# PABannier/biogpt.cpp

Measured on AMD Instinct MI355X. Metric: decode tokens/sec BioGPT Q4_0 n_ctx=1024, higher is better.
Workload: dtype int8; 1 GPU; greedy 200-token continuation of a 4-token prompt per GPU (main.cpp loop, -b 8, --top_k 1), BioGPT-base Q4_0, F32 KV cache, n_ctx=1024; 1 step = 1 continuation per rank; n_layer=24, d_model=1024, d_ff=4096, n_vocab=42384, n_predict=200, n_prompt=4, parallelism=replicas x1 (weights RCCL-broadcast once)

## Files before the change

### biogpt.cpp_amd/csrc/kernels_xpipe.hip.h

```cpp
#pragma once

#include "kernels_decode.hip.h"

namespace bgk {

typedef unsigned long long xp_u64;
typedef float xp_v4f __attribute__((ext_vector_type(4)));
#define XP_RLX __ATOMIC_RELAXED, __HIP_MEMORY_SCOPE_AGENT
constexpr uint32_t XP_SPIN_MAX = 400000u;

struct XpLayer {
    const float *ln0_w, *ln0_b, *ln1_w, *ln1_b;
    const float *bqkv, *bo, *b1, *b2;
    DevMatrix Wqkv, Wo, W1, W2;
    float *kcache, *vcache;
    unsigned long long *gx1, *gx;
};

constexpr int XP_G_QKV = 0;
constexpr int XP_G_ATT = 3072;
constexpr int XP_G_X1 = XP_G_ATT + 320;
constexpr int XP_G_H = XP_G_X1 + 1024;
constexpr int XP_G_X = XP_G_H + 1280;
constexpr int XP_G_LAYER = XP_G_X + 1024;
// ... 288 lines not shown
constexpr int XP_S_G = XP_S_PART + 256 * DEC_PS * 4;
constexpr int XP_S_LN = XP_S_G + 512;
constexpr int XP_S_BIAS = XP_S_LN + 16384;
constexpr int XP_S_CUR = XP_S_BIAS + 1536;
constexpr int XP_S_S = XP_S_CUR + 768;
constexpr int XP_S_REDF = XP_S_S + 1024;
constexpr int XP_S_REDD = XP_S_REDF + 512;
constexpr int XP_S_PV = XP_S_REDD + 128;
constexpr int XP_S_TOTAL = XP_S_PV + 8192;
static_assert(32 * DEC_PS2 <= 256 * DEC_PS, "fc2 block terms fit the shared region");
__host__ __device__ inline size_t xpipe_smem_bytes(int gelu_entries) { return XP_S_TOTAL + (size_t)gelu_entries * 2; }

template <int WT, bool EXPAND>
__device__ __forceinline__ float xp_dot(const Unit<WT> &u, const uint32_t *xq, float xd, float xs_f, int xs_i) {
    if constexpr (EXPAND) return unit_dot_settled<WT>(u, xq, xd, xs_f, xs_i);
    else return unit_dot_quant<WT>(u, xq, xd, xs_f, xs_i);
}
template <int WT, bool EXPAND>
__device__ __forceinline__ void xp_settle(Unit<WT> &u) {
    if constexpr (EXPAND) {
        settle_unit<WT>(u);
        asm volatile("" : "+v"(u.q0.x), "+v"(u.q0.y), "+v"(u.q0.z), "+v"(u.q0.w), "+v"(u.q1.x), "+v"(u.q1.y), "+v"(u.q1.z), "+v"(u.q1.w), "+v"(u.sc));
    }
}

__device__ __forceinline__ uint32_t xp_wave_sum_u32(uint32_t v) {
    int s = (int)v;
    s += dpp_i<DPP_QUAD_XOR1>(s); s += dpp_i<DPP_QUAD_XOR2>(s); s += dpp_i<DPP_ROW_HALF_MIRROR>(s); s += dpp_i<DPP_ROW_MIRROR>(s);
    return (uint32_t)((__builtin_amdgcn_readlane(s, 0) + __builtin_amdgcn_readlane(s, 16)) + (__builtin_amdgcn_readlane(s, 32) + __builtin_amdgcn_readlane(s, 48)));
}

template <int WT, int LPK, int NW, int KCAP, int ROLE, bool SPLIT, bool RES>
__device__ __forceinline__ void xp_run(const XpParams &p, unsigned char *smem, const int xcd, const int slot, const uint32_t epoch0, const int n_past0,
                                       const int n_gen0) {
    using TI = TypeInfo<WT>;
    static_assert(TI::quant && (WT != W_Q8_0 || SPLIT), "18-30 weight units per lane must fit the register file (Q8_0: 9 registers per unit: split layers)");
    static_assert(ROLE == 0 || ROLE == 1 || (ROLE == 2 && SPLIT), "0 attention head, 1 q/k/v rows, 2 (split layers) the MLP half");
    static_assert(SPLIT || TI::q81, "the producers publish Q8_0 block sums only for Q4_1 / Q5_1 (want_sum = q81): the symmetric formats need the signed units of the split form (unit_dot_settled)");
    constexpr bool ATTN = ROLE == 0;
    constexpr bool EXPAND = SPLIT;
    constexpr bool FIRST = !SPLIT || ROLE != 2, SECOND = !SPLIT || ROLE == 2;
    static_assert(LPK == 2 || LPK == 4 || LPK == 8 || LPK == 16, "lanes per key");
    static_assert(NW == 8 || NW == 16, "waves per workgroup");
    constexpr int D = 1024, DK = 64, NT = NW * 64;
    constexpr int QS = 96 / NW, OS = 16 / NW, FS = 64 / NW, F2R = 32 / NW;
    constexpr bool DUAL = SPLIT && KCAP > 256;
    constexpr int KW = DUAL ? KCAP / 2 : KCAP;
    constexpr int HI = (DUAL && ROLE == 1) ? 1 : 0;
    static_assert(KW % NW == 0 && KW <= NW * 64 / LPK, "key capacity of the launch");
    constexpr int NF4 = 16 / LPK, NV = KW / NW;
    float *const s_x = reinterpret_cast<float *>(smem + XP_S_X);
    float *const s_x1 = reinterpret_cast<float *>(smem + XP_S_X1);
    uint32_t *const s_xq = reinterpret_cast<uint32_t *>(smem + XP_S_XQ);
    float *const s_xd = reinterpret_cast<float *>(smem + XP_S_XD);
    uint32_t *const s_xs = reinterpret_cast<uint32_t *>(smem + XP_S_XS);
    double *const s_red = reinterpret_cast<double *>(smem + XP_S_RED);
    uint32_t *const s_hq = reinterpret_cast<uint32_t *>(smem + XP_S_HQ);
    float *const s_hd = reinterpret_cast<float *>(smem + XP_S_HD);
    uint32_t *const s_hs = reinterpret_cast<uint32_t *>(smem + XP_S_HS);
    float *const s_part = reinterpret_cast<float *>(smem + XP_S_PART);
    float *const s_g = reinterpret_cast<float *>(smem + XP_S_G);
    float *const s_ln = reinterpret_cast<float *>(smem + XP_S_LN);
    float *const s_bias = reinterpret_cast<float *>(smem + XP_S_BIAS);
    float *const s_cur = reinterpret_cast<float *>(smem + XP_S_CUR);
    float *const s_S = reinterpret_cast<float *>(smem + XP_S_S);
    float *const s_redf = reinterpret_cast<float *>(smem + XP_S_REDF);
    int *const s_redi = reinterpret_cast<int *>(smem + XP_S_REDF + 256);
    double *const s_redd = reinterpret_cast<double *>(smem + XP_S_REDD);
    double *const s_pv = reinterpret_cast<double *>(smem + XP_S_PV);
    uint16_t *const s_gelu = reinterpret_cast<uint16_t *>(smem + XP_S_TOTAL);
    uint32_t *const s_dead = reinterpret_cast<uint32_t *>(smem + XP_S_REDD + 96);
    uint32_t *const s_kvdead = reinterpret_cast<uint32_t *>(smem + XP_S_REDD + 64);
    uint32_t *const s_spec = reinterpret_cast<uint32_t *>(smem + XP_S_REDD + 112);
    const int t_cap = p.t_cap;
    const int n_units = SPLIT ? 2 * p.n_layer : p.n_layer;
    const int last_xcd = (n_units - 1) & 7;
    for (int tk = 0; tk < p.n_tok; tk++) {
    const uint32_t epoch = epoch0 + (uint32_t)tk;
    uint32_t etag = epoch;
    const int n_past = n_past0 + tk, T = n_past + 1;
    if (tk > 0 && __hip_atomic_load(p.ctl + 1, XP_RLX) != 0u) break;
    for (int U = xcd; U < n_units; U += 8) {
        const int L = SPLIT ? (U >> 1) : U;
        int tid = threadIdx.x;
        asm volatile("" : "+v"(tid));
        const int lane = tid & 63, wave = tid >> 6;
        const int sub = lane & 31, rsub = lane >> 5;
        const bool worker = tid < 256;
        if (tk == 0 && U == xcd && U >= 2) {
            if (tid == 0) {
                const xp_u64 *g = SPLIT ? (ROLE != 2 ? XPL(L - 1).gx1 : XPL(L - 1).gx) : XPL(L - 2).gx;
                for (uint32_t spins = 0;; spins++) {
                    if ((uint32_t)(__hip_atomic_load(g, XP_RLX) >> 32) == epoch) break;
                    if (spins >= XP_SPIN_MAX) { xp_fail(p, 3u); break; }
                    if ((spins & 255u) == 255u && __hip_atomic_load(p.ctl + 1, XP_RLX) != 0u) break;
                    __builtin_amdgcn_s_sleep(16);
                }
            }
            __syncthreads();
        }
        const XpLayerK &Y = XPL(L);
        xp_u64 *const G = p.gran + (size_t)L * XP_G_LAYER;
        constexpr bool attn_wg = ATTN || (DUAL && ROLE == 1);
        const int head = slot & 15;
        Unit<WT> wo[OS], w1[FS], w2[F2R][2];
        {
            float4 l0 = make_float4(0.f, 0.f, 0.f, 0.f), l1 = l0, l2 = l0, l3 = l0;
            if (worker) {
                if (FIRST) { l0 = xp_ldg4(Y.ln0_w, tid); l1 = xp_ldg4(Y.ln0_b, tid); }
                if (SECOND) { l2 = xp_ldg4(Y.ln1_w, tid); l3 = xp_ldg4(Y.ln1_b, tid); }
            }
            float bv = 0.0f;
            if (tid < 192) { if (FIRST) bv = ((xp_gf)Y.bqkv)[(tid >> 6) * 1024 + head * 64 + (tid & 63)]; }
            else if (tid < 224) { if (FIRST) bv = ((xp_gf)Y.bo)[slot * 32 + tid - 192]; }
            else if (tid < 352) { if (SECOND) bv = ((xp_gf)Y.b1)[slot * 128 + tid - 224]; }
            else if (tid < 384) { if (SECOND) bv = ((xp_gf)Y.b2)[slot * 32 + tid - 352]; }
            if (FIRST) {
#pragma unroll
                for (int s = 0; s < OS; s++) load_unit<WT>(wo[s], XPL_MATRIX(Y.Wo), (int64_t)(slot * 32 + s * 2 * NW + wave * 2 + rsub) * 32 + sub);
            }
            if (SECOND) {
#pragma unroll
                for (int s = 0; s < FS; s++) load_unit<WT>(w1[s], XPL_MATRIX(Y.W1), (int64_t)(slot * 128 + s * 2 * NW + wave * 2 + rsub) * 32 + sub);
#pragma unroll
                for (int r = 0; r < F2R; r++)
#pragma unroll
                    for (int it = 0; it < 2; it++) load_unit<WT>(w2[r][it], XPL_MATRIX(Y.W2), (int64_t)(slot * 32 + wave * F2R + r) * 128 + lane + 64 * it);
            }
            if (worker) {
                if (FIRST) { reinterpret_cast<float4 *>(s_ln)[tid] = l0; reinterpret_cast<float4 *>(s_ln + 1024)[tid] = l1; }
                if (SECOND) { reinterpret_cast<float4 *>(s_ln + 2048)[tid] = l2; reinterpret_cast<float4 *>(s_ln + 3072)[tid] = l3; }
            }
            if (tid < 384) s_bias[tid] = bv;
            if constexpr (EXPAND) {
                if (FIRST) {
#pragma unroll
                    for (int s = 0; s < OS; s++) xp_settle<WT, EXPAND>(wo[s]);
                }
                if (SECOND) {
#pragma unroll
                    for (int s = 0; s < FS; s++) xp_settle<WT, EXPAND>(w1[s]);
#pragma unroll
                    for (int r = 0; r < F2R; r++) { xp_settle<WT, EXPAND>(w2[r][0]); xp_settle<WT, EXPAND>(w2[r][1]); }
                }
            }
        }
        auto layer_input = [&]() -> float4 {
            float4 xv = make_float4(0.f, 0.f, 0.f, 0.f);
            if (L == 0) {
                int tok;
                const bool emb_fast = XPK(tok_emb.type) == WT && XPK(pos_emb.type) == WT;
                uint32_t pq = 0u, psc = 0u, pqh = 0u;
                if (emb_fast && worker) xp_row4_request<WT>(XPK_MATRIX(pos_emb), n_past + 2, tid, pq, psc, pqh);
                auto sample_prev = [&]() __attribute__((always_inline)) -> int {
                    float bv = -INFINITY;
                    int bi = 0x7fffffff;
                    {
                        uint32_t v[4] = {0u, 0u, 0u, 0u};
                        const bool a0 = tid < XPK(lm_blocks), a1 = tid + NT < XPK(lm_blocks);
                        const uint32_t prev = epoch - 1u;
                        for (uint32_t spins = 0; !RES || etag != 0u; spins++) {
                            bool ok = true;
                            if (a0) {
                                const xp_u64 x0 = __hip_atomic_load(XPK(samp) + tid, XP_RLX), x1 = __hip_atomic_load(XPK(samp) + 1024 + tid, XP_RLX);
                                v[0] = (uint32_t)x0; v[1] = (uint32_t)x1;
                                ok &= (uint32_t)(x0 >> 32) == prev && (uint32_t)(x1 >> 32) == prev;
                            }
                            if (a1) {
                                const xp_u64 x0 = __hip_atomic_load(XPK(samp) + tid + NT, XP_RLX), x1 = __hip_atomic_load(XPK(samp) + 1024 + tid + NT, XP_RLX);
                                v[2] = (uint32_t)x0; v[3] = (uint32_t)x1;
                                ok &= (uint32_t)(x0 >> 32) == prev && (uint32_t)(x1 >> 32) == prev;
                            }
                            if (__all(ok)) break;
                            if (spins >= XP_SPIN_MAX) { if (lane == 0) xp_fail(p, 4u); if (RES) etag = 0u; break; }
                            if ((spins & (RES ? 255u : 1023u)) == (RES ? 255u : 1023u) && __any(__hip_atomic_load(p.ctl + 1, XP_RLX) != 0u)) { if (RES) etag = 0u; break; }
                            
                        }
                        if (a0) { bv = __uint_as_float(v[0]); bi = (int)v[1]; }
                        if (a1) {
                            const float ov = __uint_as_float(v[2]);
                            const int oi = (int)v[3];
                            if (ov > bv || (ov == bv && oi < bi)) { bv = ov; bi = oi; }
                        }
                    }
                    xp_argmax_wave(bv, bi);
                    if (lane == 0) { s_redf[wave] = bv; s_redi[wave] = bi; }
                    __syncthreads();
                    bv = s_redf[0]; bi = s_redi[0];
#pragma unroll
                    for (int w = 1; w < NW; w++)
                        if (s_redf[w] > bv || (s_redf[w] == bv && s_redi[w] < bi)) { bv = s_redf[w]; bi = s_redi[w]; }
                    if (bi < 0 || bi >= XPK(n_vocab)) bi = 0;
                    return bi;
                };
                if (RES && p.resident != 0 && tk == 0 && slot == 0 && tid == 0) { s_spec[0] = (uint32_t)XPK(res_spec0); s_spec[1] = 0xffffffffu; }
                if (RES && p.resident != 0 && tk > 0) {
                    xp_u64 *const gt = XPK(samp) + 2048;
                    if (slot == 0) {
                        unsigned long long *const wl4 = ((XPK(res_dbg) & 32) && XPK(wall) && tid == 0) ? XPK(wall) + 32768 + (size_t)((XPK(mbox_seq0) + (uint32_t)tk) & 4095u) * 4 : nullptr;
                        if (wl4) wl4[0] = wall_clock64();
                        const uint32_t want = XPK(mbox_seq0) + (uint32_t)tk;
                        auto wait_post = [&](uint32_t seq, int np, int &spec) __attribute__((always_inline)) -> int {
                            const xp_u64 *mb = reinterpret_cast<const xp_u64 *>(XPK(mbox)) + (size_t)(seq & 63u) * 4;
                            const unsigned long long t0 = wall_clock64();
                            for (;;) {
                                const xp_u64 w = __hip_atomic_load(mb, __ATOMIC_RELAXED, __HIP_MEMORY_SCOPE_SYSTEM);
                                if ((uint32_t)(w >> 40) == (seq & 0xffffffu)) {
                                    const int tv = (int)(w & 0xffffffu), pn = (int)((w >> 24) & 0x1fffu);
                                    spec = (int)((w >> 37) & 1u);
                                    return (pn == np && tv < XPK(n_vocab)) ? tv : -1;
                                }
                                if (wall_clock64() - t0 > (unsigned long long)XPK(idle_ticks)) return -1;
                                if (__hip_atomic_load(p.ctl + 1, XP_RLX) != 0u) return -1;
                                if (!(XPK(res_dbg) & 2)) __builtin_amdgcn_s_sleep(4);
                            }
                        };
                        if (tid == 0) {
                            const int pending = (int)s_spec[1];
                            int unused = 0;
                            s_spec[2] = (etag != 0u && (pending < 0 || wait_post(want - 1u, n_past - 1, unused) == pending)) ? 1u : 0u;
                        }
                        const int guess = sample_prev();
                        __syncthreads();
                        if (wl4) wl4[1] = wall_clock64();
                        if (tid == 0 && etag != 0u) {
                            int spec = (int)s_spec[0];
                            const bool ahead = (int)s_spec[1] >= 0 || spec != 0;
                            int got = -1;
                            if (s_spec[2] != 0u) {
                                if (XPK(spec_rec)) __hip_atomic_store(XPK(spec_rec), ((unsigned long long)want << 32) | (unsigned long long)(uint32_t)guess, __ATOMIC_RELAXED, __HIP_MEMORY_SCOPE_SYSTEM);
                                got = ahead ? guess : wait_post(want, n_past, spec);
                            }
                            if (got >= 0) {
                                xp_put_local(gt, epoch, (uint32_t)got);
                                xp_put(gt + 1, epoch, 1u);
                                s_spec[0] = (uint32_t)spec; s_spec[1] = ahead ? (uint32_t)guess : 0xffffffffu;
                            } else xp_quit(p);
                            if ((XPK(res_dbg) & 32) && XPK(wall)) XPK(wall)[(size_t)(want & 4095u) * 2] = wall_clock64();
                            if (wl4) wl4[2] = wall_clock64();
                        }
                    }
                    uint32_t v[1];
                    xp_sweep_q<RES, 1>(gt, true, epoch, v, p, etag);
                    tok = (int)v[0];
                    if (tok < 0 || tok >= XPK(n_vocab)) tok = 0;
                } else if (tk > 0) {
                    tok = sample_prev();
                    if (slot == 0 && tid == 0) {
                        int32_t *tokens = state_tokens(XPK(st));
                        const int g = n_gen0 + tk;
                        if (g < XPK(n_positions)) tokens[XPK(n_positions) + g] = tok;
                        tokens[0] = tok;
                    }
                    __syncthreads();
                } else if (XPK(tok_src) == 2) {
                    float bv = -INFINITY;
                    int bi = 0x7fffffff;
                    for (int k = tid; k < XPK(nparts); k += NT) {
                        const float v = XPK(pmax_val)[k];
                        const int ix = XPK(pmax_idx)[k];
                        if (v > bv || (v == bv && ix < bi)) { bv = v; bi = ix; }
                    }
    #pragma unroll
                    for (int off = 32; off > 0; off >>= 1) {
                        const float ov = __shfl_xor(bv, off, 64);
                        const int oi = __shfl_xor(bi, off, 64);
                        if (ov > bv || (ov == bv && oi < bi)) { bv = ov; bi = oi; }
                    }
                    if (lane == 0) { s_redf[wave] = bv; s_redi[wave] = bi; }
                    __syncthreads();
                    bv = s_redf[0]; bi = s_redi[0];
    #pragma unroll
                    for (int w = 1; w < NW; w++)
                        if (s_redf[w] > bv || (s_redf[w] == bv && s_redi[w] < bi)) { bv = s_redf[w]; bi = s_redi[w]; }
                    tok = bi;
                    if (tok < 0 || tok >= XPK(n_vocab)) tok = 0;
                    if (slot == 0 && tid == 0) {
                        int32_t *tokens = state_tokens(XPK(st));
                        const int g = n_gen0;
                        if (g < XPK(n_positions)) tokens[XPK(n_positions) + g] = tok;
                        tokens[0] = tok;
                    }
                } else {
                    tok = (RES && p.resident != 0) ? XPK(res_tok0) : state_tokens(XPK(st))[0];
                }
                if (slot == 0) XP_TAIL(tk, 5);
                if (worker) {
                    float e[4];
                    if (emb_fast) {
                        uint32_t tq, tsc, tqh;
                        xp_row4_request<WT>(XPK_MATRIX(tok_emb), tok, tid, tq, tsc, tqh);
                        float te[4], pe[4];
                        xp_row4_values<WT>(pq, psc, pqh, tid, pe);
                        xp_row4_values<WT>(tq, tsc, tqh, tid, te);
    #pragma unroll
                        for (int j = 0; j < 4; j++) e[j] = __fadd_rn(__fmul_rn(te[j], XPK(embed_scale)), pe[j]);
                    } else {
    #pragma unroll
                        for (int j = 0; j < 4; j++)
                            e[j] = __fadd_rn(__fmul_rn(dequant_elem(XPK_MATRIX(tok_emb), tok, 4 * tid + j), XPK(embed_scale)), dequant_elem(XPK_MATRIX(pos_emb), n_past + 2, 4 * tid + j));
                    }
                    xv = make_float4(e[0], e[1], e[2], e[3]);
                }
            } else if (wave < 4) {
                uint32_t v[4];
                xp_sweep_q<RES, 4, 256, true>(XPL(L - 1).gx + tid, true, epoch, v, p, etag);
                xv = make_float4(__uint_as_float(v[0]), __uint_as_float(v[1]), __uint_as_float(v[2]), __uint_as_float(v[3]));
            }
            if (RES && wave < 4 && lane == 0) { s_dead[wave] = (etag == 0u) ? 1u : 0u; }
            return xv;
        };
        if constexpr (FIRST) {
        constexpr bool MERGE = SPLIT && KCAP <= 128;
        if (!attn_wg && MERGE) {
            const float4 xv = layer_input();
            if (worker) reinterpret_cast<float4 *>(s_x)[tid] = xv;
            XP_WALL(0);
        }
        if (!attn_wg && !MERGE) {
            constexpr int Q0 = (KCAP <= 192) ? QS / 3 : 0;
            Unit<WT> wqkv[QS];
#pragma unroll
            for (int s = Q0; s < QS; s++) {
                const int jj = s * 2 * NW + wave * 2 + rsub;
                load_unit<WT>(wqkv[s], XPL_MATRIX(Y.Wqkv), (int64_t)((jj >> 6) * 1024 + head * 64 + (jj & 63)) * 32 + sub);
            }
#pragma unroll
            for (int s = Q0; s < QS; s++) xp_settle<WT, EXPAND>(wqkv[s]);
            const float4 xv = layer_input();
            XP_WALL(0);
            float4 lnw = xv, lnb = xv;
            if (worker) {
                reinterpret_cast<float4 *>(s_x)[tid] = xv;
                lnw = reinterpret_cast<const float4 *>(s_ln)[tid]; lnb = reinterpret_cast<const float4 *>(s_ln + 1024)[tid];
            }
            ln4_q8_1024<TI::q81, TI::q81>(xv, lnw, lnb, p.eps, s_red, s_xq, s_xd, s_xs);
            XP_WALL(6);
            uint32_t ax[8];
            const uint4 a = *reinterpret_cast<const uint4 *>(s_xq + sub * 8), b = *reinterpret_cast<const uint4 *>(s_xq + sub * 8 + 4);
            ax[0] = a.x; ax[1] = a.y; ax[2] = a.z; ax[3] = a.w; ax[4] = b.x; ax[5] = b.y; ax[6] = b.z; ax[7] = b.w;
            const float axd = s_xd[sub];
            const uint32_t axs = s_xs[sub];
            float *const part = s_part + wave * 2 * QS * DEC_PS;
#pragma unroll
            for (int s = Q0; s < QS; s++) part[(s * 2 + rsub) * DEC_PS + sub] = xp_dot<WT, EXPAND>(wqkv[s], ax, axd, __uint_as_float(axs), (int)axs);
            __builtin_amdgcn_fence(__ATOMIC_RELEASE, "wavefront");
            __builtin_amdgcn_wave_barrier();
            __builtin_amdgcn_fence(__ATOMIC_ACQUIRE, "wavefront");
            if (lane >= 2 * Q0 && lane < 2 * QS) {
                const int jj = (lane >> 1) * 2 * NW + wave * 2 + (lane & 1);
                float v = __fadd_rn(s_bias[jj], sum32_in_order(part + lane * DEC_PS));
                const int which = jj >> 6, d = jj & 63;
                if (which == 0) v = __fmul_rn(v, p.q_scale);
                xp_put_local(G + XP_G_QKV + which * 1024 + head * 64 + d, etag, __float_as_uint(v));
                if (which != 0 && (!RES || (etag != 0u && (s_dead[0] | s_dead[1] | s_dead[2] | s_dead[3]) == 0u))) {
                    float *kc_ = Y.kcache, *vc_ = Y.vcache;
                    asm volatile("" : "+s"(kc_), "+s"(vc_));
                    ((__attribute__((address_space(1))) float *)((which == 1) ? kc_ : vc_))[((size_t)head * p.P + n_past) * DK + d] = v;
                }
            }
            XP_WALL(1);
        }
        if (attn_wg) {
            float4 kr[NF4];
            float vr[NV];
            const int ksub = tid & (LPK - 1), kidx = tid / LPK;
            const int dd = tid & (DK - 1), sl = tid >> 6;
            {
                constexpr bool KV_SC1 = !MERGE;
                const float *kb = Y.kcache + (size_t)head * p.P * DK, *vb = Y.vcache + (size_t)head * p.P * DK;
                const __amdgpu_buffer_rsrc_t krs = xp_kv_rsrc(kb, p.P * DK * 4), vrs = xp_kv_rsrc(vb, p.P * DK * 4);
                if (KV_SC1 || kidx < t_cap) {
#pragma unroll
                    for (int m = 0; m < NF4; m++) kr[m] = xp_kv_load4<KV_SC1>(krs, kb, ((HI * KW + kidx) * (DK / 4) + ksub + LPK * m) * 4);
                } else {
#pragma unroll
                    for (int m = 0; m < NF4; m++) kr[m] = make_float4(0.f, 0.f, 0.f, 0.f);
                }
#pragma unroll
                for (int k = 0; k < NV; k++) {
                    const int j = HI * KW + sl + NW * k;
                    vr[k] = (KV_SC1 || j < t_cap) ? xp_kv_load1<KV_SC1>(vrs, vb, j * DK + dd) : 0.0f;
                }
            }
            if constexpr (MERGE) {
                Unit<WT> wqkv[QS];
#pragma unroll
                for (int s = 0; s < QS; s++) {
                    const int jj = s * 2 * NW + wave * 2 + rsub;
                    load_unit<WT>(wqkv[s], XPL_MATRIX(Y.Wqkv), (int64_t)((jj >> 6) * 1024 + head * 64 + (jj & 63)) * 32 + sub);
                }
#pragma unroll
                for (int s = 0; s < QS; s++) xp_settle<WT, EXPAND>(wqkv[s]);
                const float4 xv = layer_input();
                XP_WALL(0);
                if (L == 0 && slot == 0) { asm volatile("" :: "v"(xv.x)); XP_TAIL(tk, 6); }
                float4 lnw = xv, lnb = xv;
                if (worker) {
// ... 338 lines not shown
            if (lane < 2 * OS) {
                const int lr = (lane >> 1) * 2 * NW + wave * 2 + (lane & 1), row = slot * 32 + lr;
                const float v = __fadd_rn(__fadd_rn(sum32_in_order(part + lane * DEC_PS), s_bias[192 + lr]), s_x[row]);
                if (SPLIT) xp_put(Y.gx1 + xp_col_slot(row), etag, __float_as_uint(v));
                else xp_put_local(Y.gx1 + xp_col_slot(row), etag, __float_as_uint(v));
            }
        }
        XP_WALL(3);
        }
        if constexpr (SECOND) {
        float4 x1v = make_float4(0.f, 0.f, 0.f, 0.f), lnw = x1v, lnb = x1v;
        if (wave < 4) {
            uint32_t v[4];
            xp_sweep_q<RES, 4, 256, true>(Y.gx1 + tid, true, epoch, v, p, etag);
            x1v = make_float4(__uint_as_float(v[0]), __uint_as_float(v[1]), __uint_as_float(v[2]), __uint_as_float(v[3]));
            reinterpret_cast<float4 *>(s_x1)[tid] = x1v;
            XP_WALL(9);
            lnw = reinterpret_cast<const float4 *>(s_ln + 2048)[tid]; lnb = reinterpret_cast<const float4 *>(s_ln + 3072)[tid];
        }
        ln4_q8_1024<TI::q81, TI::q81>(x1v, lnw, lnb, p.eps, s_red, s_xq, s_xd, s_xs);
        XP_WALL(10);
        {
            uint32_t ax[8];
            const uint4 a = *reinterpret_cast<const uint4 *>(s_xq + sub * 8), b = *reinterpret_cast<const uint4 *>(s_xq + sub * 8 + 4);
            ax[0] = a.x; ax[1] = a.y; ax[2] = a.z; ax[3] = a.w; ax[4] = b.x; ax[5] = b.y; ax[6] = b.z; ax[7] = b.w;
            const float axd = s_xd[sub];
            const uint32_t axs = s_xs[sub];
            float *const part = s_part + wave * 2 * FS * DEC_PS;
#pragma unroll
            for (int s = 0; s < FS; s++) part[(s * 2 + rsub) * DEC_PS + sub] = xp_dot<WT, EXPAND>(w1[s], ax, axd, __uint_as_float(axs), (int)axs);
            __builtin_amdgcn_fence(__ATOMIC_RELEASE, "wavefront");
            __builtin_amdgcn_wave_barrier();
            __builtin_amdgcn_fence(__ATOMIC_ACQUIRE, "wavefront");
            if (lane < 2 * FS) {
                const int jr = (lane >> 1) * 2 * NW + wave * 2 + (lane & 1);
                const float v = __fadd_rn(s_bias[224 + jr], sum32_in_order(part + lane * DEC_PS));
                const uint32_t ix = f2h(v), neg = ix - 0x8000u;
                uint16_t g16;
                if (ix < (uint32_t)p.gelu_p) g16 = s_gelu[ix];
                else if (ix <= 0x7C00u) g16 = (p.gelu_p > 0) ? (uint16_t)ix : p.gelu_tab[ix];
                else if (neg < (uint32_t)p.gelu_n) g16 = s_gelu[p.gelu_p + neg];
                else if (neg < 0x7C00u && p.gelu_n > 0) g16 = (uint16_t)p.gelu_z;
                else g16 = p.gelu_tab[ix];
                s_g[jr] = h2f(g16);
            }
        }
        __syncthreads();
        XP_WALL(11);
        if (tid < 128) {
            int8_t q8; float d8; uint32_t s8;
            q8_block32(s_g[tid], TI::q81, q8, d8, s8, TI::q81);
            const uint32_t packed = xp_pack4(q8);
            const int blk = slot * 4 + (tid >> 5);
            if ((tid & 3) == 0) xp_put_local(G + XP_G_H + slot * 32 + (tid >> 2), etag, packed);
            if ((tid & 31) == 0) { xp_put_local(G + XP_G_H + 1024 + blk, etag, __float_as_uint(d8)); if (TI::q81) xp_put_local(G + XP_G_H + 1152 + blk, etag, s8); }
        }
        XP_WALL(4);
        {
            constexpr int NQ = 1024 / NT;
            uint32_t v[NQ + 1];
#pragma unroll
            for (int k = 0; k <= NQ; k++) v[k] = 0u;
            const xp_u64 *g = G + XP_G_H + tid;
            const bool tail = tid < (TI::q81 ? 256 : 128);
            for (uint32_t spins = 0; !RES || etag != 0u; spins++) {
                bool ok = true;
#pragma unroll
                for (int k = 0; k < NQ; k++) {
                    const xp_u64 a = __hip_atomic_load(g + k * NT, XP_RLX);
                    v[k] = (uint32_t)a;
                    ok &= (uint32_t)(a >> 32) == epoch;
                }
                if (tail) {
                    const xp_u64 a = __hip_atomic_load(g + 1024, XP_RLX);
                    v[NQ] = (uint32_t)a;
                    ok &= (uint32_t)(a >> 32) == epoch;
                }
                if (__all(ok)) break;
                if (spins >= XP_SPIN_MAX) { if (lane == 0) xp_fail(p, 1u); if (RES) etag = 0u; break; }
                if ((spins & (RES ? 255u : 1023u)) == (RES ? 255u : 1023u) && __any(__hip_atomic_load(p.ctl + 1, XP_RLX) != 0u)) { if (RES) etag = 0u; break; }
                
            }
#pragma unroll
            for (int k = 0; k < NQ; k++) s_hq[tid + k * NT] = v[k];
            if (tid < 128) s_hd[tid] = __uint_as_float(v[NQ]);
            else if (tid < 256) s_hs[tid - 128] = v[NQ];
        }
        __syncthreads();
        XP_WALL(12);
        {
            float *const part = s_part + wave * F2R * DEC_PS2;
#pragma unroll
            for (int it = 0; it < 2; it++) {
                const int u = lane + 64 * it;
                uint32_t ax[8];
                const uint4 a = *reinterpret_cast<const uint4 *>(s_hq + u * 8), b = *reinterpret_cast<const uint4 *>(s_hq + u * 8 + 4);
                ax[0] = a.x; ax[1] = a.y; ax[2] = a.z; ax[3] = a.w; ax[4] = b.x; ax[5] = b.y; ax[6] = b.z; ax[7] = b.w;
                const float axd = s_hd[u];
                const uint32_t axs = s_hs[u];
#pragma unroll
                for (int r = 0; r < F2R; r++) part[r * DEC_PS2 + u] = xp_dot<WT, EXPAND>(w2[r][it], ax, axd, __uint_as_float(axs), (int)axs);
            }
            __builtin_amdgcn_fence(__ATOMIC_RELEASE, "wavefront");
            __builtin_amdgcn_wave_barrier();
            __builtin_amdgcn_fence(__ATOMIC_ACQUIRE, "wavefront");
            if (lane < F2R) {
                const float4 *p4 = reinterpret_cast<const float4 *>(part + lane * DEC_PS2);
                float sumf = 0.0f;
#pragma unroll
                for (int b0 = 0; b0 < 32; b0 += 8) {
                    float4 t[8];
#pragma unroll
                    for (int j = 0; j < 8; j++) t[j] = p4[b0 + j];
#pragma unroll
                    for (int j = 0; j < 8; j++) {
                        sumf = __fadd_rn(sumf, t[j].x); sumf = __fadd_rn(sumf, t[j].y);
                        sumf = __fadd_rn(sumf, t[j].z); sumf = __fadd_rn(sumf, t[j].w);
                    }
                }
                const int lr = wave * F2R + lane, row = slot * 32 + lr;
                const float v = __fadd_rn(__fadd_rn(sumf, s_bias[352 + lr]), s_x1[row]);
                xp_put(Y.gx + xp_col_slot(row), etag, __float_as_uint(v));
                if (L == p.n_layer - 1) XPK(x_final)[row] = v;
            }
        }
        XP_WALL(5);
        if (L == p.n_layer - 1 && slot == 0) XP_TAIL(tk, 0);
        }
        __syncthreads();
    }
    const int lm_rank = xp_lm_rank(xcd, slot, n_units);
    if (p.lm != 0 && lm_rank >= 0 && lm_rank * 4 < XPK(lm_blocks)) {
        int tid = threadIdx.x;
        asm volatile("" : "+v"(tid));
        const int lane = tid & 63, wave = tid >> 6;
        const int sub = lane & 31, rsub = lane >> 5;
        const bool worker = tid < 256;
        constexpr int LMS = 128 / NW;
        const int row0 = lm_rank * 256;
        const bool alt = RES && p.resident != 0 && ((XPK(mbox_seq0) + (uint32_t)tk) & 1u) != 0u;
        float *const lg_dev = alt ? XPK(logits_alt) : XPK(logits);
        float *const lg_host = alt ? XPK(logits_host_alt) : XPK(logits_host);
        Unit<WT> wl[LMS];
#pragma unroll
        for (int s = 0; s < LMS; s++) {
            const int row = row0 + s * 2 * NW + wave * 2 + rsub;
            if (row < XPK(n_vocab)) load_unit<WT>(wl[s], XPK_MATRIX(Wlm), (int64_t)row * 32 + sub);
            else { wl[s].q0 = make_uint4(0u, 0u, 0u, 0u); wl[s].q1 = wl[s].q0; wl[s].sc = 0u; wl[s].qh = 0u; }
        }
#pragma unroll
        for (int s = 0; s < LMS; s++) xp_settle<WT, EXPAND>(wl[s]);
        float4 xv = make_float4(0.f, 0.f, 0.f, 0.f), lnw = xv, lnb = xv;
        if (worker) { lnw = reinterpret_cast<const float4 *>(XPK(lm_ln_w))[tid]; lnb = reinterpret_cast<const float4 *>(XPK(lm_ln_b))[tid]; }
        if (RES && p.resident != 0 && tk > 0 && !(XPK(res_dbg) & 64)) {
            uint32_t go[1];
            xp_sweep_q<RES, 1>(XPK(samp) + 2049, lane == 0, epoch, go, p, etag);
        }
        if (wave < 4) {
            uint32_t v[4];
            xp_sweep_q<RES, 4, 256, true>(XPL(p.n_layer - 1).gx + tid, true, epoch, v, p, etag);
            xv = make_float4(__uint_as_float(v[0]), __uint_as_float(v[1]), __uint_as_float(v[2]), __uint_as_float(v[3]));
            if (lm_rank == 0) XP_TAIL(tk, 1);
        }
        ln4_q8_1024<TI::q81, TI::q81>(xv, lnw, lnb, p.eps, s_red, s_xq, s_xd, s_xs);
        if (lm_rank == 0) XP_TAIL(tk, 2);
        uint32_t ax[8];
        const uint4 a = *reinterpret_cast<const uint4 *>(s_xq + sub * 8), b = *reinterpret_cast<const uint4 *>(s_xq + sub * 8 + 4);
        ax[0] = a.x; ax[1] = a.y; ax[2] = a.z; ax[3] = a.w; ax[4] = b.x; ax[5] = b.y; ax[6] = b.z; ax[7] = b.w;
        const float axd = s_xd[sub];
        const uint32_t axs = s_xs[sub];
        float *const part = s_part + wave * 2 * LMS * DEC_PS;
#pragma unroll
        for (int s = 0; s < LMS; s++) part[(s * 2 + rsub) * DEC_PS + sub] = xp_dot<WT, EXPAND>(wl[s], ax, axd, __uint_as_float(axs), (int)axs);
        __builtin_amdgcn_fence(__ATOMIC_RELEASE, "wavefront");
        __builtin_amdgcn_wave_barrier();
        __builtin_amdgcn_fence(__ATOMIC_ACQUIRE, "wavefront");
        float best_val = -INFINITY;
        int best_idx = 0x7fffffff;
        if (lane < 2 * LMS) {
            const int row = row0 + (lane >> 1) * 2 * NW + wave * 2 + (lane & 1);
            if (row < XPK(n_vocab)) {
                const float v = sum32_in_order(part + lane * DEC_PS);
                if constexpr (RES) s_S[row - row0] = v;
                else { XPK(logits)[row] = v; if (XPK(logits_host)) XPK(logits_host)[row] = v; }
                best_val = v; best_idx = row;
            }
        }
        if (lm_rank == 0) XP_TAIL(tk, 3);
        static_assert(64 / NW == 8 || 64 / NW == 4, "finisher lanes per block");
        xp_argmax_dpp<DPP_QUAD_XOR1>(best_val, best_idx); xp_argmax_dpp<DPP_QUAD_XOR2>(best_val, best_idx);
        if (64 / NW == 8) xp_argmax_dpp<DPP_ROW_HALF_MIRROR>(best_val, best_idx);
        constexpr int LPB = 64 / NW;
        if (lane < 2 * LMS && (lane & (LPB - 1)) == 0) { s_redf[(lane / LPB) * NW + wave] = best_val; s_redi[(lane / LPB) * NW + wave] = best_idx; }
        bool row_ok = true;
        if constexpr (RES) row_ok = __syncthreads_and(etag != 0u);
        else __syncthreads();
        if (RES && lg_host && wave == 1 && row_ok) {
            const int r = row0 + 4 * lane;
            if (XPK(res_dbg) & 4) {
            } else if (r + 3 < XPK(n_vocab)) {
                const xp_v4f v4 = *reinterpret_cast<const xp_v4f *>(s_S + 4 * lane);
                asm volatile("global_store_dwordx4 %0, %1, off sc0 sc1" :: "v"(lg_host + r), "v"(v4) : "memory");
                *reinterpret_cast<xp_v4f *>(lg_dev + r) = v4;
            } else {
                for (int j = r; j < XPK(n_vocab); j++) { __hip_atomic_store(lg_host + j, s_S[j - row0], __ATOMIC_RELAXED, __HIP_MEMORY_SCOPE_SYSTEM); lg_dev[j] = s_S[j - row0]; }
            }
            if (p.resident != 0) {
                if (lane < 4 && lm_rank * 4 + lane < XPK(lm_blocks)) {
                    float bm = s_redf[lane * NW];
#pragma unroll
                    for (int w = 1; w < NW; w++) bm = fmaxf(bm, s_redf[lane * NW + w]);
                    __hip_atomic_store(lg_host + xp_blockmax_offset(XPK(n_vocab)) + lm_rank * 4 + lane, bm, __ATOMIC_RELAXED, __HIP_MEMORY_SCOPE_SYSTEM);
                }
                if (!(XPK(res_dbg) & 1)) asm volatile("s_waitcnt vmcnt(0)" ::: "memory");
                if (lane == 0) __hip_atomic_store(XPK(done_host) + lm_rank, XPK(mbox_seq0) + (uint32_t)tk, __ATOMIC_RELAXED, __HIP_MEMORY_SCOPE_SYSTEM);
                if ((XPK(res_dbg) & 32) && XPK(wall) && lane == 0 && lm_rank == 0) XPK(wall)[(size_t)((XPK(mbox_seq0) + (uint32_t)tk) & 4095u) * 2 + 1] = wall_clock64();
                if ((XPK(res_dbg) & 32) && XPK(wall) && lane == 0) XPK(wall)[8192 + (size_t)((XPK(mbox_seq0) + (uint32_t)tk) & 63u) * 256 + lm_rank] = wall_clock64();
            }
        }
        if (tid < 4) {
            float bv = s_redf[tid * NW];
            int bi = s_redi[tid * NW];
#pragma unroll
            for (int w = 1; w < NW; w++) {
                const float ov = s_redf[tid * NW + w];
                const int oi = s_redi[tid * NW + w];
                if (ov > bv || (ov == bv && oi < bi)) { bv = ov; bi = oi; }
            }
            const int blk = lm_rank * 4 + tid;
            if (blk < XPK(lm_blocks)) {
                if (RES && !row_ok) {}
                else if (RES && alt) { XPK(pmax_alt_val)[blk] = bv; XPK(pmax_alt_idx)[blk] = bi; }
                else { XPK(pmax_out_val)[blk] = bv; XPK(pmax_out_idx)[blk] = bi; }
                if (tk + 1 < p.n_tok) {
                    xp_put(XPK(samp) + blk, etag, __float_as_uint(bv));
                    xp_put(XPK(samp) + 1024 + blk, etag, (uint32_t)bi);
                }
                if (RES && (XPK(res_dbg) & 32) && XPK(wall) && blk == 0) XPK(wall)[32768 + (size_t)((XPK(mbox_seq0) + (uint32_t)tk) & 4095u) * 4 + 3] = wall_clock64();
            }
        }
        if (lm_rank == 0) XP_TAIL(tk, 4);
        __syncthreads();
    }
    }
    if (threadIdx.x == 0) {
        if (xcd == last_xcd && slot == 0) {
            if (epoch0 + (uint32_t)p.n_tok > 0xF0000000u) xp_fail(p, 5u);
            __hip_atomic_store(p.ctl, epoch0 + (uint32_t)p.n_tok, XP_RLX);
            __hip_atomic_store(p.ctl + 2, __hip_atomic_load(p.ctl + 2, XP_RLX) + 1u, XP_RLX);
        }
        if (xcd == (last_xcd == 1 ? 2 : 1) && slot == 0 && p.adv != 0) { XPK(st)->n_past = n_past0 + p.n_tok; XPK(st)->n_gen = n_gen0 + p.n_tok; }
    }
}

template <int WT, int LPK, int NW, int KCAP, bool SPLIT, bool RES = false>
__global__ __launch_bounds__(NW * 64) void dec_xpipe_kernel(const XpParams p) {
    using TI = TypeInfo<WT>;
    static_assert(TI::quant && (WT != W_Q8_0 || SPLIT), "Q8_0 (9 registers per weight unit) runs with split layers");
    static_assert(LPK == 2 || LPK == 4 || LPK == 8 || LPK == 16, "lanes per key");
    static_assert(NW == 8 || NW == 16, "waves per workgroup");
    constexpr int D = 1024, DK = 64, NT = NW * 64;
    constexpr int QS = 96 / NW, OS = 16 / NW, FS = 64 / NW, F2R = 32 / NW;
    static_assert(KCAP % NW == 0 && (KCAP > 256 ? KCAP / 2 : KCAP) <= NW * 64 / LPK, "key capacity of the launch");
    constexpr int NF4 = 16 / LPK, NV = (KCAP > 256 ? KCAP / 2 : KCAP) / NW;
    extern __shared__ __attribute__((aligned(16))) unsigned char smem[];
    float *const s_x = reinterpret_cast<float *>(smem + XP_S_X);
    float *const s_x1 = reinterpret_cast<float *>(smem + XP_S_X1);
    uint32_t *const s_xq = reinterpret_cast<uint32_t *>(smem + XP_S_XQ);
    float *const s_xd = reinterpret_cast<float *>(smem + XP_S_XD);
    uint32_t *const s_xs = reinterpret_cast<uint32_t *>(smem + XP_S_XS);
    double *const s_red = reinterpret_cast<double *>(smem + XP_S_RED);
    uint32_t *const s_hq = reinterpret_cast<uint32_t *>(smem + XP_S_HQ);
    float *const s_hd = reinterpret_cast<float *>(smem + XP_S_HD);
    uint32_t *const s_hs = reinterpret_cast<uint32_t *>(smem + XP_S_HS);
    float *const s_part = reinterpret_cast<float *>(smem + XP_S_PART);
    float *const s_g = reinterpret_cast<float *>(smem + XP_S_G);
    float *const s_ln = reinterpret_cast<float *>(smem + XP_S_LN);
    float *const s_bias = reinterpret_cast<float *>(smem + XP_S_BIAS);
    float *const s_cur = reinterpret_cast<float *>(smem + XP_S_CUR);
    float *const s_S = reinterpret_cast<float *>(smem + XP_S_S);
    float *const s_redf = reinterpret_cast<float *>(smem + XP_S_REDF);
    int *const s_redi = reinterpret_cast<int *>(smem + XP_S_REDF + 256);
    double *const s_redd = reinterpret_cast<double *>(smem + XP_S_REDD);
    double *const s_pv = reinterpret_cast<double *>(smem + XP_S_PV);
    uint16_t *const s_gelu = reinterpret_cast<uint16_t *>(smem + XP_S_TOTAL);

    const uint32_t epoch0 = __hip_atomic_load(p.ctl, XP_RLX);
    if (threadIdx.x == 0) {
        const uint32_t xcc = __builtin_amdgcn_s_getreg(20 | (3 << 11)) & 7u;
        const uint32_t t = __hip_atomic_fetch_add(p.ctl + 8 + xcc, 1u, XP_RLX);
        s_redi[0] = (int)xcc;
        s_redi[1] = (int)(t - 32u * (__hip_atomic_load(p.ctl + 2, XP_RLX) - 1u));
    }
    __syncthreads();
    const int xcd = __builtin_amdgcn_readfirstlane(s_redi[0]), slot = __builtin_amdgcn_readfirstlane(s_redi[1]);
    __syncthreads();
    if ((unsigned)slot >= 32u) { if (threadIdx.x == 0) xp_fail(p, 2u); return; }
    const int n_past0 = (RES && p.resident != 0) ? p.res_n_past0 : p.st->n_past, n_gen0 = p.st->n_gen;
    const int t_cap = p.t_cap;

    if (!SPLIT || (xcd & 1)) {
        const uint4 *src = reinterpret_cast<const uint4 *>(p.gelu_tab);
        const int np8 = p.gelu_p / 8, nn8 = p.gelu_n / 8;
        for (int i = threadIdx.x; i < np8; i += NT) reinterpret_cast<uint4 *>(s_gelu)[i] = src[i];
        for (int i = threadIdx.x; i < nn8; i += NT) reinterpret_cast<uint4 *>(s_gelu + p.gelu_p)[i] = src[0x8000 / 8 + i];
    }
    if (SPLIT && !(xcd & 1) && (slot < 16 || KCAP > 256) && p.exp_n > 0) {
        const uint4 *src = reinterpret_cast<const uint4 *>(p.exp_tab + 0x8000);
        for (int i = threadIdx.x; i < p.exp_n / 8; i += NT) reinterpret_cast<uint4 *>(s_gelu)[i] = src[i];
    }
#ifdef XP_ONLY_ROLE
    xp_run<WT, LPK, NW, KCAP, XP_ONLY_ROLE, true, RES>(p, smem, xcd, slot, epoch0, n_past0, n_gen0);
#else
    if constexpr (SPLIT) {
        if (xcd & 1) { xp_run<WT, LPK, NW, KCAP, 2, true, RES>(p, smem, xcd, slot, epoch0, n_past0, n_gen0); return; }
    }
    if (slot < 16) xp_run<WT, LPK, NW, KCAP, 0, SPLIT, RES>(p, smem, xcd, slot, epoch0, n_past0, n_gen0);
    else xp_run<WT, LPK, NW, KCAP, 1, SPLIT, RES>(p, smem, xcd, slot, epoch0, n_past0, n_gen0);
#endif
}

struct XpProbe { unsigned long long *addr; int32_t src, dst; };
__global__ void xp_hop_probe_kernel(const XpProbe *pr, int n, int reps, uint32_t *tickets, unsigned long long *ticks, uint32_t *err) {
    if (threadIdx.x != 0) return;
    const int xcc = (int)(__builtin_amdgcn_s_getreg(20 | (3 << 11)) & 7u);
    const uint32_t role = __hip_atomic_fetch_add(tickets + xcc, 1u, XP_RLX);
    if (role > 1u) return;
    for (int i = 0; i < n; i++) {
        const XpProbe q = pr[i];
        if ((role == 0u ? q.src : q.dst) != xcc) continue;
        xp_u64 *X = q.addr, *Y = q.addr + 1;
        const xp_u64 base = 0xFFFF000000000000ull | ((xp_u64)i << 16);
        const unsigned long long t0 = wall_clock64();
        for (int r = 1; r <= reps; r++) {
            const xp_u64 want = base + (xp_u64)r;
            if (role == 0u) __hip_atomic_store(X, want, XP_RLX);
            const xp_u64 *w = role == 0u ? Y : X;
            for (uint32_t spins = 0; __hip_atomic_load(w, XP_RLX) != want; spins++)
                if (spins > XP_SPIN_MAX || ((spins & 1023u) == 1023u && __hip_atomic_load(err, XP_RLX) != 0u)) { __hip_atomic_store(err, 1u, XP_RLX); return; }
            if (role == 1u) __hip_atomic_store(Y, want, XP_RLX);
        }
        if (role == 0u) ticks[i] = wall_clock64() - t0;
    }
}

__global__ void xp_probe_kernel(uint32_t *out) {
    if (threadIdx.x == 0) out[blockIdx.x] = __builtin_amdgcn_s_getreg(20 | (3 << 11)) & 15u;
}

}
```

Measured before the change: 4186 tokens/s.

## Pre-reduce LM-head argmax per workgroup and publish before logits stores

Each LM-head workgroup now reduces its four block maxima with DPP quad shuffles and publishes a single (value, index) pair per workgroup to the sampling mailbox, instead of one pair per block. The publish is moved ahead of the global/host logits stores, so the next token's consumer can start sooner. The consumer sampler reads a quarter as many mailbox slots, one per thread, which shortens its spin-poll. Kernel arguments are cached in locals, and profile hook tail markers are added. This assumes lm_blocks lines up with groups of four per workgroup.

```diff
diff --git a/biogpt.cpp_amd/csrc/kernels_xpipe.hip.h b/biogpt.cpp_amd/csrc/kernels_xpipe.hip.h
--- a/biogpt.cpp_amd/csrc/kernels_xpipe.hip.h
+++ b/biogpt.cpp_amd/csrc/kernels_xpipe.hip.h
@@ -464,36 +464,31 @@
                 const bool emb_fast = XPK(tok_emb.type) == WT && XPK(pos_emb.type) == WT;
                 uint32_t pq = 0u, psc = 0u, pqh = 0u;
                 if (emb_fast && worker) xp_row4_request<WT>(XPK_MATRIX(pos_emb), n_past + 2, tid, pq, psc, pqh);
+                const int n_vocab_k = XPK(n_vocab);
                 auto sample_prev = [&]() __attribute__((always_inline)) -> int {
                     float bv = -INFINITY;
                     int bi = 0x7fffffff;
                     {
-                        uint32_t v[4] = {0u, 0u, 0u, 0u};
-                        const bool a0 = tid < XPK(lm_blocks), a1 = tid + NT < XPK(lm_blocks);
+                        const xp_u64 *const sg = XPK(samp) + tid;
+                        const bool a0 = tid < ((XPK(lm_blocks) + 3) >> 2);
                         const uint32_t prev = epoch - 1u;
+                        uint32_t v0 = 0u, v1 = 0u;
                         for (uint32_t spins = 0; !RES || etag != 0u; spins++) {
                             bool ok = true;
                             if (a0) {
-                                const xp_u64 x0 = __hip_atomic_load(XPK(samp) + tid, XP_RLX), x1 = __hip_atomic_load(XPK(samp) + 1024 + tid, XP_RLX);
-                                v[0] = (uint32_t)x0; v[1] = (uint32_t)x1;
-                                ok &= (uint32_t)(x0 >> 32) == prev && (uint32_t)(x1 >> 32) == prev;
+                                const xp_u64 x0 = __hip_atomic_load((xp_gq)sg, XP_RLX), x1 = __hip_atomic_load((xp_gq)sg + 1024, XP_RLX);
+                                v0 = (uint32_t)x0; v1 = (uint32_t)x1;
+                                ok = (uint32_t)(x0 >> 32) == prev && (uint32_t)(x1 >> 32) == prev;
                             }
-                            if (a1) {
-                                const xp_u64 x0 = __hip_atomic_load(XPK(samp) + tid + NT, XP_RLX), x1 = __hip_atomic_load(XPK(samp) + 1024 + tid + NT, XP_RLX);
-                                v[2] = (uint32_t)x0; v[3] = (uint32_t)x1;
-                                ok &= (uint32_t)(x0 >> 32) == prev && (uint32_t)(x1 >> 32) == prev;
-                            }
+#ifdef BIOGPT_HIP_PROFILE_HOOKS
+                            if (spins == 0u && slot == 0) { asm volatile("" :: "v"(v0), "v"(v1)); XP_TAIL(tk, 11); }
+#endif
                             if (__all(ok)) break;
                             if (spins >= XP_SPIN_MAX) { if (lane == 0) xp_fail(p, 4u); if (RES) etag = 0u; break; }
                             if ((spins & (RES ? 255u : 1023u)) == (RES ? 255u : 1023u) && __any(__hip_atomic_load(p.ctl + 1, XP_RLX) != 0u)) { if (RES) etag = 0u; break; }
-                            
                         }
-                        if (a0) { bv = __uint_as_float(v[0]); bi = (int)v[1]; }
-                        if (a1) {
-                            const float ov = __uint_as_float(v[2]);
-                            const int oi = (int)v[3];
-                            if (ov > bv || (ov == bv && oi < bi)) { bv = ov; bi = oi; }
-                        }
+                        if (slot == 0) XP_TAIL(tk, 12);
+                        if (a0) { bv = __uint_as_float(v0); bi = (int)v1; }
                     }
                     xp_argmax_wave(bv, bi);
                     if (lane == 0) { s_redf[wave] = bv; s_redi[wave] = bi; }
@@ -502,7 +497,8 @@
 #pragma unroll
                     for (int w = 1; w < NW; w++)
                         if (s_redf[w] > bv || (s_redf[w] == bv && s_redi[w] < bi)) { bv = s_redf[w]; bi = s_redi[w]; }
-                    if (bi < 0 || bi >= XPK(n_vocab)) bi = 0;
+                    if (bi < 0 || bi >= n_vocab_k) bi = 0;
+                    if (slot == 0) XP_TAIL(tk, 13);
                     return bi;
                 };
                 if (RES && p.resident != 0 && tk == 0 && slot == 0 && tid == 0) { s_spec[0] = (uint32_t)XPK(res_spec0); s_spec[1] = 0xffffffffu; }
@@ -555,7 +551,7 @@
                     uint32_t v[1];
                     xp_sweep_q<RES, 1>(gt, true, epoch, v, p, etag);
                     tok = (int)v[0];
-                    if (tok < 0 || tok >= XPK(n_vocab)) tok = 0;
+                    if (tok < 0 || tok >= n_vocab_k) tok = 0;
                 } else if (tk > 0) {
                     tok = sample_prev();
                     if (slot == 0 && tid == 0) {
@@ -1200,6 +1196,9 @@
         for (int s = 0; s < LMS; s++) xp_settle<WT, EXPAND>(wl[s]);
         float4 xv = make_float4(0.f, 0.f, 0.f, 0.f), lnw = xv, lnb = xv;
         if (worker) { lnw = reinterpret_cast<const float4 *>(XPK(lm_ln_w))[tid]; lnb = reinterpret_cast<const float4 *>(XPK(lm_ln_b))[tid]; }
+        const int n_vocab_k = XPK(n_vocab), lm_blocks_k = XPK(lm_blocks);
+        xp_u64 *const samp_k = XPK(samp);
+        const bool more = tk + 1 < p.n_tok;
         if (RES && p.resident != 0 && tk > 0 && !(XPK(res_dbg) & 64)) {
             uint32_t go[1];
             xp_sweep_q<RES, 1>(XPK(samp) + 2049, lane == 0, epoch, go, p, etag);
@@ -1223,14 +1222,14 @@
         __builtin_amdgcn_fence(__ATOMIC_RELEASE, "wavefront");
         __builtin_amdgcn_wave_barrier();
         __builtin_amdgcn_fence(__ATOMIC_ACQUIRE, "wavefront");
-        float best_val = -INFINITY;
+        float best_val = -INFINITY, row_val = 0.0f;
         int best_idx = 0x7fffffff;
         if (lane < 2 * LMS) {
             const int row = row0 + (lane >> 1) * 2 * NW + wave * 2 + (lane & 1);
-            if (row < XPK(n_vocab)) {
+            if (row < n_vocab_k) {
                 const float v = sum32_in_order(part + lane * DEC_PS);
                 if constexpr (RES) s_S[row - row0] = v;
-                else { XPK(logits)[row] = v; if (XPK(logits_host)) XPK(logits_host)[row] = v; }
+                else row_val = v;
                 best_val = v; best_idx = row;
             }
         }
@@ -1243,6 +1242,36 @@
         bool row_ok = true;
         if constexpr (RES) row_ok = __syncthreads_and(etag != 0u);
         else __syncthreads();
+        if (lm_rank == 0) XP_TAIL(tk, 8);
+        float blk_val = -INFINITY;
+        int blk_idx = 0x7fffffff;
+        if (tid < 4) {
+            blk_val = s_redf[tid * NW];
+            blk_idx = s_redi[tid * NW];
+#pragma unroll
+            for (int w = 1; w < NW; w++) {
+                const float ov = s_redf[tid * NW + w];
+                const int oi = s_redi[tid * NW + w];
+                if (ov > blk_val || (ov == blk_val && oi < blk_idx)) { blk_val = ov; blk_idx = oi; }
+            }
+        }
+        if (more) {
+            float wg_val = blk_val;
+            int wg_idx = blk_idx;
+            xp_argmax_dpp<DPP_QUAD_XOR1>(wg_val, wg_idx); xp_argmax_dpp<DPP_QUAD_XOR2>(wg_val, wg_idx);
+            if (tid == 0) {
+                xp_put(samp_k + lm_rank, etag, __float_as_uint(wg_val));
+                xp_put(samp_k + 1024 + lm_rank, etag, (uint32_t)wg_idx);
+            }
+        }
+        if (lm_rank == 0) XP_TAIL(tk, 9);
+        if constexpr (!RES) {
+            if (lane < 2 * LMS) {
+                const int row = row0 + (lane >> 1) * 2 * NW + wave * 2 + (lane & 1);
+                if (row < n_vocab_k) { XPK(logits)[row] = row_val; if (XPK(logits_host)) XPK(logits_host)[row] = row_val; }
+            }
+        }
+        if (lm_rank == 0) XP_TAIL(tk, 10);
         if (RES && lg_host && wave == 1 && row_ok) {
             const int r = row0 + 4 * lane;
             if (XPK(res_dbg) & 4) {
@@ -1267,23 +1296,11 @@
             }
         }
         if (tid < 4) {
-            float bv = s_redf[tid * NW];
-            int bi = s_redi[tid * NW];
-#pragma unroll
-            for (int w = 1; w < NW; w++) {
-                const float ov = s_redf[tid * NW + w];
-                const int oi = s_redi[tid * NW + w];
-                if (ov > bv || (ov == bv && oi < bi)) { bv = ov; bi = oi; }
-            }
             const int blk = lm_rank * 4 + tid;
-            if (blk < XPK(lm_blocks)) {
+            if (blk < lm_blocks_k) {
                 if (RES && !row_ok) {}
-                else if (RES && alt) { XPK(pmax_alt_val)[blk] = bv; XPK(pmax_alt_idx)[blk] = bi; }
-                else { XPK(pmax_out_val)[blk] = bv; XPK(pmax_out_idx)[blk] = bi; }
-                if (tk + 1 < p.n_tok) {
-                    xp_put(XPK(samp) + blk, etag, __float_as_uint(bv));
-                    xp_put(XPK(samp) + 1024 + blk, etag, (uint32_t)bi);
-                }
+                else if (RES && alt) { XPK(pmax_alt_val)[blk] = blk_val; XPK(pmax_alt_idx)[blk] = blk_idx; }
+                else { XPK(pmax_out_val)[blk] = blk_val; XPK(pmax_out_idx)[blk] = blk_idx; }
                 if (RES && (XPK(res_dbg) & 32) && XPK(wall) && blk == 0) XPK(wall)[32768 + (size_t)((XPK(mbox_seq0) + (uint32_t)tk) & 4095u) * 4 + 3] = wall_clock64();
             }
         }
```

Measured after the change: 4184 tokens/s. Within noise of the previous version (-0.1%).
